# erlgo/openair4G

Measured on AMD Instinct MI355X. Metric: DL subframes/sec (20 MHz, 2x2, 64-QAM), higher is better.
Workload: dtype int16; 1 GPU; dlsim 20 MHz 2x2 TM3 (LARGE_CDD) 64-QAM MCS19x2CW, 2x14 IDFT-2048; config_id=C3, global_batch=8192, subframe_index=7, full_grid=False, parallelism=subframe-sharded x1

## Files before the change

include/oai4g.h:

```cpp
#ifndef OAI4G_H
#define OAI4G_H

#include <stddef.h>
#include <stdint.h>

#ifdef __cplusplus
extern "C" {
#endif

#define OAI4G_LTE_NULL 2
#define OAI4G_NSOFT 1827072
#define OAI4G_MAX_SEGMENTS 16
#define OAI4G_MAX_CHANNEL_BITS (14 * 1200 * 6)
#define OAI4G_D_BYTES (96 + 12 + 3 + 3 * 6144)
#define OAI4G_W_BYTES (3 * 6144 + 96)

enum { OAI4G_SISO = 0, OAI4G_ALAMOUTI = 1, OAI4G_LARGE_CDD = 2 };
enum { OAI4G_CYCLIC_PREFIX = 0, OAI4G_CYCLIC_SUFFIX = 1, OAI4G_ZEROS = 2, OAI4G_NONE = 3 };

typedef struct {
  uint16_t N_RB_DL;
  uint16_t Nid_cell;
  uint8_t Ncp;
  uint8_t nushift;
// ... 23 lines not shown
  uint32_t format;
  uint8_t dci_pdu[8];
} oai4g_dci_alloc_t;

typedef struct {
  uint32_t TBS;
  uint32_t B;
  uint8_t *b;
  uint8_t *c[OAI4G_MAX_SEGMENTS];
  uint32_t RTC[OAI4G_MAX_SEGMENTS];
  uint8_t round;
  uint8_t mcs;
  uint8_t rvidx;
  uint8_t mimo_mode;
  uint32_t rb_alloc[4];
  uint16_t nb_rb;
  uint8_t *e;
  uint8_t *d[OAI4G_MAX_SEGMENTS];
  uint8_t *w[OAI4G_MAX_SEGMENTS];
  uint32_t C, Cminus, Cplus, Kminus, Kplus, F;
  uint8_t Nl;
  uint8_t Nlayers;
  uint8_t first_layer;
} oai4g_dl_harq_t;

typedef struct {
  uint16_t rnti;
  uint8_t current_harq_pid;
  uint8_t Mdlharq;
  uint8_t Kmimo;
  int16_t sqrt_rho_a;
  int16_t sqrt_rho_b;
  oai4g_dl_harq_t *harq_processes[8];
} oai4g_dlsch_t;

int oai4g_init(void);
const char *oai4g_last_error(void);
int oai4g_device_name(char *buf, int len);

int oai4g_init_frame_parms(oai4g_frame_parms_t *fp, uint16_t N_RB_DL, uint16_t Nid_cell, uint8_t Ncp,
                           uint8_t nb_antennas_tx, uint8_t mode1_flag, uint8_t frame_type);
uint8_t oai4g_get_Qm(uint8_t mcs);
int oai4g_get_G(const oai4g_frame_parms_t *fp, uint16_t nb_rb, const uint32_t *rb_alloc, uint8_t mod_order,
                uint8_t Nl, uint8_t num_pdcch_symbols, int frame, uint8_t subframe);
uint8_t oai4g_get_Qm_ul(uint8_t mcs);
uint8_t oai4g_get_I_TBS(uint8_t mcs);
uint8_t oai4g_get_I_TBS_UL(uint8_t mcs);
uint32_t oai4g_tbs_bits(uint8_t I_TBS, uint16_t nb_rb);
uint32_t oai4g_get_TBS_DL(uint8_t mcs, uint16_t nb_rb);
uint32_t oai4g_get_TBS_UL(uint8_t mcs, uint16_t nb_rb);
oai4g_dlsch_t *oai4g_new_dlsch(uint8_t Kmimo, uint8_t Mdlharq, uint8_t N_RB_DL);
void oai4g_free_dlsch(oai4g_dlsch_t *dlsch);
uint32_t oai4g_lte_gold_generic(uint32_t *x1, uint32_t *x2, uint8_t reset);

uint32_t oai4g_crc24a(const uint8_t *in, int bitlen);
uint32_t oai4g_crc24b(const uint8_t *in, int bitlen);
int oai4g_lte_segmentation(const uint8_t *input_buffer, uint8_t **output_buffers, uint32_t B, uint32_t *C,
                           uint32_t *Cplus, uint32_t *Cminus, uint32_t *Kplus, uint32_t *Kminus, uint32_t *F);
void oai4g_threegpplte_turbo_encoder(const uint8_t *input, uint16_t input_length_bytes, uint8_t *output,
                                     uint8_t F, uint16_t interleaver_f1, uint16_t interleaver_f2);
uint32_t oai4g_sub_block_interleaving_turbo(uint32_t D, uint8_t *d, uint8_t *w);
uint32_t oai4g_lte_rate_matching_turbo(uint32_t RTC, uint32_t G, const uint8_t *w, uint8_t *e, uint8_t C,
                                       uint32_t Nsoft, uint8_t Mdlharq, uint8_t Kmimo, uint8_t rvidx,
                                       uint8_t Qm, uint8_t Nl, uint8_t r, uint8_t nb_rb, uint8_t m);
int oai4g_dlsch_encoding(uint8_t *a, const oai4g_frame_parms_t *frame_parms, uint8_t num_pdcch_symbols,
                         oai4g_dlsch_t *dlsch, int frame, uint8_t subframe);
void oai4g_dlsch_scrambling(const oai4g_frame_parms_t *frame_parms, int mbsfn_flag, oai4g_dlsch_t *dlsch, int G,
                            uint8_t q, uint8_t Ns);
int oai4g_dlsch_modulation(int32_t **txdataF, int16_t amp, uint32_t subframe_offset,
                           const oai4g_frame_parms_t *frame_parms, uint8_t num_pdcch_symbols,
                           oai4g_dlsch_t *dlsch0, oai4g_dlsch_t *dlsch1);
void oai4g_PHY_ofdm_mod(const int32_t *input, int32_t *output, uint8_t log2fftsize, uint8_t nb_symbols,
                        uint16_t nb_prefix_samples, int etype);
void oai4g_normal_prefix_mod(const int32_t *txdataF, int32_t *txdata, uint8_t nsymb,
                             const oai4g_frame_parms_t *frame_parms);
void oai4g_do_OFDM_mod(int32_t **txdataF, int32_t **txdata, uint32_t frame, uint16_t next_slot,
                       const oai4g_frame_parms_t *frame_parms);
void oai4g_generate_pilots(int32_t **txdataF, int16_t amp, const oai4g_frame_parms_t *frame_parms, uint16_t Ntti);
int oai4g_lte_dl_cell_spec(int32_t *output, int16_t amp, const oai4g_frame_parms_t *frame_parms, uint8_t Ns,
                           uint8_t l, uint8_t p);
int oai4g_idft(int log2n, const int16_t *x, int16_t *y, int scale);
void oai4g_idft2048(const int16_t *x, int16_t *y, int scale);
void oai4g_idft1024(const int16_t *x, int16_t *y, int scale);
void oai4g_idft512(const int16_t *x, int16_t *y, int scale);
void oai4g_idft256(const int16_t *x, int16_t *y, int scale);
void oai4g_idft128(const int16_t *x, int16_t *y, int scale);
void oai4g_idft64(const int16_t *x, int16_t *y, int scale);

void oai4g_generate_pcfich_reg_mapping(const oai4g_frame_parms_t *frame_parms, uint16_t pcfich_reg[4],
                                       uint8_t *pcfich_first_reg_idx);
int oai4g_generate_pcfich(uint8_t num_pdcch_symbols, int16_t amp, const oai4g_frame_parms_t *frame_parms,
                          int32_t **txdataF, uint8_t subframe);

uint8_t oai4g_get_mi(const oai4g_frame_parms_t *frame_parms, uint8_t subframe);
uint16_t oai4g_get_nquad(uint8_t num_pdcch_symbols, const oai4g_frame_parms_t *frame_parms, uint8_t mi);
uint16_t oai4g_get_nCCE(uint8_t num_pdcch_symbols, const oai4g_frame_parms_t *frame_parms, uint8_t mi);
uint8_t oai4g_get_num_pdcch_symbols(uint8_t num_dci, const oai4g_dci_alloc_t *dci_alloc,
                                    const oai4g_frame_parms_t *frame_parms, uint8_t subframe);
int oai4g_generate_phich_reg_mapping(const oai4g_frame_parms_t *frame_parms, uint16_t phich_reg[56][3]);
void oai4g_init_nCCE_table(void);
int oai4g_get_nCCE_offset(uint8_t L, int nCCE, int common_dci, uint16_t rnti, uint8_t subframe);
uint8_t oai4g_generate_dci_top(uint8_t num_ue_spec_dci, uint8_t num_common_dci, const oai4g_dci_alloc_t *dci_alloc,
                               uint32_t n_rnti, int16_t amp, const oai4g_frame_parms_t *frame_parms,
                               int32_t **txdataF, uint32_t subframe);

int oai4g_rx_pdsch_siso(const oai4g_frame_parms_t *frame_parms, const int32_t *rxdataF, const int32_t *dl_ch_estimates,
// ... 234 lines not shown
```

openair4g_amd/__init__.py:

```python
import ctypes
import os

import numpy as np

_HERE = os.path.dirname(os.path.abspath(__file__))
LIB_PATH = os.path.join(_HERE, "lib", "libopenair4g_amd.so")

LTE_NULL = 2
NSOFT = 1827072
MAX_SEGMENTS = 16
MAX_CHANNEL_BITS = 14 * 1200 * 6
D_BYTES = 96 + 12 + 3 + 3 * 6144
W_BYTES = 3 * 6144 + 96
SISO, ALAMOUTI, LARGE_CDD = 0, 1, 2
CYCLIC_PREFIX = 0


class OAI4GError(RuntimeError):
    pass


u8p = ctypes.POINTER(ctypes.c_uint8)


# ... 243 lines not shown
                                                 ctypes.c_uint8, ctypes.c_uint32, ctypes.c_uint8]),
    "oai4g_ul_config_destroy": (None, [ctypes.c_void_p]),
    "oai4g_ul_config_C": (ctypes.c_int, [ctypes.c_void_p]),
    "oai4g_ul_config_E": (ctypes.c_uint32, [ctypes.c_void_p, ctypes.c_int]),
    "oai4g_ul_config_G_offset": (ctypes.c_uint32, [ctypes.c_void_p, ctypes.c_int]),
    "oai4g_ul_decode_batch": (ctypes.c_int, [ctypes.c_void_p, ctypes.c_int, ctypes.c_void_p, ctypes.c_size_t,
                                             ctypes.c_void_p, ctypes.c_size_t, ctypes.c_void_p, ctypes.c_void_p]),
    "oai4g_ul_config_w_entries": (ctypes.c_size_t, [ctypes.c_void_p]),
    "oai4g_ul_decode_batch_harq": (ctypes.c_int, [ctypes.c_void_p, ctypes.c_int, ctypes.c_void_p, ctypes.c_size_t,
                                                  ctypes.c_void_p, ctypes.c_size_t, ctypes.c_uint8, ctypes.c_uint8,
                                                  ctypes.c_void_p, ctypes.c_size_t, ctypes.c_void_p, ctypes.c_void_p]),
    "oai4g_dft": (ctypes.c_int, [ctypes.c_int, ctypes.c_void_p, ctypes.c_void_p, ctypes.c_int]),
    "oai4g_dft2048": (None, [ctypes.c_void_p, ctypes.c_void_p, ctypes.c_int]),
    "oai4g_dft1024": (None, [ctypes.c_void_p, ctypes.c_void_p, ctypes.c_int]),
    "oai4g_dft512": (None, [ctypes.c_void_p, ctypes.c_void_p, ctypes.c_int]),
    "oai4g_dft256": (None, [ctypes.c_void_p, ctypes.c_void_p, ctypes.c_int]),
    "oai4g_dft128": (None, [ctypes.c_void_p, ctypes.c_void_p, ctypes.c_int]),
    "oai4g_dft64": (None, [ctypes.c_void_p, ctypes.c_void_p, ctypes.c_int]),
    "oai4g_slot_fep_offset": (ctypes.c_int64, [ctypes.POINTER(FrameParms), ctypes.c_uint8, ctypes.c_uint8,
                                               ctypes.c_int, ctypes.c_int]),
    "oai4g_slot_fep": (ctypes.c_int, [ctypes.POINTER(ctypes.c_void_p), ctypes.POINTER(ctypes.c_void_p),
                                      ctypes.POINTER(FrameParms), ctypes.c_uint8, ctypes.c_uint8, ctypes.c_uint8,
                                      ctypes.c_int, ctypes.c_int]),
    "oai4g_fep_batch": (ctypes.c_int, [ctypes.POINTER(FrameParms), ctypes.c_int, ctypes.c_int, ctypes.c_void_p,
                                       ctypes.c_void_p, ctypes.c_void_p]),
    "oai4g_tx_config_create": (ctypes.c_void_p, [ctypes.POINTER(TxParams)]),
    "oai4g_tx_config_destroy": (None, [ctypes.c_void_p]),
    "oai4g_tx_G": (ctypes.c_uint32, [ctypes.c_void_p, ctypes.c_int, ctypes.c_int]),
    "oai4g_tx_ebits_words": (ctypes.c_uint32, [ctypes.c_void_p]),
    "oai4g_tx_iq_samples": (ctypes.c_uint32, [ctypes.c_void_p]),
    "oai4g_tx_workspace_bytes": (ctypes.c_size_t, [ctypes.c_void_p, ctypes.c_int]),
    "oai4g_tx_batch": (ctypes.c_int, [ctypes.c_void_p, ctypes.c_int, ctypes.c_void_p, ctypes.c_void_p,
                                      ctypes.c_void_p, ctypes.c_void_p]),
    "oai4g_tx_batch_timed": (ctypes.c_int, [ctypes.c_void_p, ctypes.c_int, ctypes.c_void_p, ctypes.c_void_p,
                                            ctypes.c_void_p, ctypes.c_void_p, ctypes.POINTER(ctypes.c_float)]),
    "oai4g_tx_encode": (ctypes.c_int, [ctypes.c_void_p, ctypes.c_int, ctypes.c_void_p, ctypes.c_void_p,
                                       ctypes.c_void_p]),
    "oai4g_tx_modulate": (ctypes.c_int, [ctypes.c_void_p, ctypes.c_int, ctypes.c_void_p, ctypes.c_void_p,
                                         ctypes.c_void_p]),
    "oai4g_tx_mod_nosat": (ctypes.c_int, [ctypes.c_void_p]),
    "oai4g_diag_encode_phase_ms": (ctypes.c_int, [ctypes.c_void_p, ctypes.c_int, ctypes.c_void_p, ctypes.c_void_p,
                                                  ctypes.c_int, ctypes.c_int, ctypes.POINTER(ctypes.c_float)]),
    "oai4g_diag_encode_occupancy": (ctypes.c_int, [ctypes.c_void_p, ctypes.POINTER(ctypes.c_int),
                                                   ctypes.POINTER(ctypes.c_size_t)]),
    "oai4g_diag_stream": (ctypes.c_int, [ctypes.c_void_p, ctypes.c_void_p, ctypes.c_size_t, ctypes.c_int,
                                         ctypes.c_void_p]),
    "oai4g_dev_alloc": (ctypes.c_void_p, [ctypes.c_size_t]),
    "oai4g_dev_free": (None, [ctypes.c_void_p]),
    "oai4g_memcpy_h2d": (ctypes.c_int, [ctypes.c_void_p, ctypes.c_void_p, ctypes.c_size_t]),
    "oai4g_memcpy_d2h": (ctypes.c_int, [ctypes.c_void_p, ctypes.c_void_p, ctypes.c_size_t]),
    "oai4g_memset_d": (ctypes.c_int, [ctypes.c_void_p, ctypes.c_int, ctypes.c_size_t]),
    "oai4g_sync": (ctypes.c_int, []),
    "oai4g_fill_payload": (ctypes.c_int, [ctypes.c_void_p, ctypes.c_size_t, ctypes.c_uint64, ctypes.c_void_p]),
}


def load_library(path=None):
    global _lib
    if _lib is not None:
        return _lib
    path = path or os.environ.get("OAI4G_LIB") or LIB_PATH
    if not os.path.exists(path):
        raise OAI4GError(f"HIP library not built: {path} (run __graft_entry__.build())")
    lib = ctypes.CDLL(path)
    for name, (res, args) in _SIGS.items():
        fn = getattr(lib, name)
        fn.restype = res
        fn.argtypes = args
    _lib = lib
    return lib


def exported_symbols():
    return sorted(_SIGS)


def lib():
    return load_library()


def init():
    L = lib()
    if L.oai4g_init() != 0:
        raise OAI4GError(L.oai4g_last_error().decode())
    return L


def _check(ok):
    if not ok:
        raise OAI4GError(lib().oai4g_last_error().decode())


def _ptr(a):
    return ctypes.c_void_p(a.ctypes.data)


def device_name():
    L = init()
    buf = ctypes.create_string_buffer(256)
    _check(L.oai4g_device_name(buf, 256) == 0)
    return buf.value.decode()


def frame_parms(N_RB_DL, Nid_cell=0, Ncp=0, nb_antennas_tx=1, mode1_flag=1, frame_type=0):
    fp = FrameParms()
    _check(lib().oai4g_init_frame_parms(ctypes.byref(fp), N_RB_DL, Nid_cell, Ncp, nb_antennas_tx, mode1_flag,
# ... 1005 lines not shown
```

openair4g_amd/csrc/oai4g_encode.hip:

```cpp
#include "oai4g_internal.h"

struct rsc_tables_t {
  uint8_t next[8][16];
  uint8_t par[8][16];
  uint8_t apow[8][8];
  uint32_t hz;
  uint32_t zs[8];
  uint32_t fm[3];
};

static constexpr uint8_t rsc_step_c(uint8_t u, uint8_t s, uint8_t *out)
{
  *out = (uint8_t)((u ^ (s >> 2) ^ (s >> 1)) & 1);
  return (uint8_t)((((u << 2) ^ (s >> 1)) ^ ((s >> 1) << 2) ^ (s << 2)) & 7);
}

static constexpr rsc_tables_t make_rsc_tables()
{
  rsc_tables_t t{};
  for (int s = 0; s < 8; s++)
    for (int nib = 0; nib < 16; nib++) {
      uint8_t st = (uint8_t)s, p = 0;
      for (int b = 0; b < 4; b++) {
        uint8_t o = 0;
// ... 585 lines not shown
  if (DEBUG && dbg.b)
    for (uint32_t i = tid; i < Ab + 3; i += nth) dbg.b[i] = tbb[i];
  if (stop_phase <= 1) return;

  for (uint32_t i = tid; i < C * 3 * 4; i += nth) {
    const uint32_t slot = i >> 2, r = slot / 3;
    const uint32_t w = (r < n0 ? kw0 : kw1) + (i & 3u);
    if (w < sw) strm[slot * sw + w] = 0u;
  }
  auto unit_of = [&](uint32_t i, uint32_t &r, uint32_t &j, uint32_t &K, uint32_t &ki) {
    ki = i >= u0 ? 1u : 0u;
    const uint32_t ii = ki ? i - u0 : i, kw = ki ? kw1 : kw0;
    const uint32_t rr = __umul24(ii, ki ? km1 : km0) >> 20;
    j = ii - __umul24(rr, kw);
    r = ki ? n0 + rr : rr;
    K = ki ? kk1 : kk0;
  };
  for (uint32_t i = tid; i < nw; i += nth) {
    uint32_t r, j, K, ki;
    unit_of(i, r, j, K, ki);
    uint32_t fill, ncopy, s0;
    seg_of(r, fill, ncopy, s0);
    const uint32_t i0 = 4 * j;
    uint32_t le;
    if (i0 >= fill) {
      const uint32_t a = s0 + i0 - fill, wi = a >> 2;
      le = __builtin_amdgcn_alignbit(tbw[wi + 1], tbw[wi], (a & 3u) * 8u);
      const int sh = (int)(fill + ncopy) - (int)i0;
      if (C > 1 && sh < 4) {
        const uint32_t crcle = __builtin_bswap32(crcs[1 + r] << 8);
        const uint32_t cw32 = (uint32_t)(((uint64_t)crcle << (8 * (sh + 4))) >> 32);
        le = (sh > 0 ? le & (0xffffffffu >> (32 - 8 * sh)) : 0u) | cw32;
      }
    } else {
      const uint32_t crcb = C > 1 ? crcs[1 + r] : 0;
      le = 0;
      for (uint32_t q = 0; q < 4; q++) {
        const uint32_t ib = i0 + q;
        uint32_t byte = 0;
        if (ib < fill) byte = 0;
        else if (ib < fill + ncopy) byte = tbb[s0 + ib - fill];
        else if (C > 1 && ib < fill + ncopy + 3) byte = (crcb >> (8 * (2 - (ib - fill - ncopy)))) & 0xffu;
        le |= byte << (8 * q);
      }
    }
    uint32_t wv = bytes_to_seq(le);
    if (32 * (j + 1) > K) wv &= (1u << (K - 32 * j)) - 1u;
    strm[r * 3 * sw + j] = wv;
  }
  __syncthreads();
  if (stop_phase <= 2) return;

  uint32_t *ilv = lds_base;
  for (uint32_t r = 0; r < C; r++) {
    const uint32_t K = r < n0 ? kk0 : kk1, Kw = (K + 31) >> 5, Q = K >> 2, io = r < n0 ? r * kw0 : u0 + (r - n0) * kw1;
    const uint32_t *sys = strm + r * 3 * sw;
    for (uint32_t w = tid; w < Kw; w += nth) ilv[io + w] = 0u;
    const uint32_t ng = (Q + 31) >> 5, nbw = (Q + 7) >> 3;
    for (uint32_t g = tid; g < ng; g += nth) {
      uint32_t P[4];
#pragma unroll
      for (uint32_t q = 0; q < 4; q++) {
        const uint32_t src = 32 * g + q * Q, wi = src >> 5;
        const uint32_t lo = sys[wi], hi = wi + 1 < Kw ? sys[wi + 1] : 0u;
        uint32_t v = __builtin_amdgcn_alignbit(hi, lo, src);
        if (src + 32 > K) v |= sys[0] << (K - src);
        P[q] = v;
      }
#pragma unroll
      for (uint32_t jb = 0; jb < 4; jb++) {
        const uint32_t t01 = __builtin_amdgcn_perm(P[1], P[0], 0x0c0c0000u | jb | ((4 + jb) << 8));
        const uint32_t t23 = __builtin_amdgcn_perm(P[3], P[2], 0x00000c0cu | (jb << 16) | ((4 + jb) << 24));
        if (4 * g + jb < nbw) strm[(r * 3 + 1) * sw + 4 * g + jb] = t01 | t23;
      }
    }
  }
  __syncthreads();
  {
    const bool s3a = __builtin_amdgcn_readfirstlane(cw.qpp_s3[0]) != 0, s3b = __builtin_amdgcn_readfirstlane(cw.qpp_s3[1]) != 0;
    for (uint32_t i = tid; i < nw; i += nth) {
      uint32_t r, j, K, ki;
      unit_of(i, r, j, K, ki);
      const uint32_t Q = K >> 2;
      const uint4 e4 = *(const uint4 *)&cw.qpp_tab[ki][4 * j];
      const uint32_t ew[4] = {e4.x, e4.y, e4.z, e4.w};
      const uint32_t *b8 = strm + (r * 3 + 1) * sw;
      uint32_t acc = 0;
#pragma unroll
      for (int b = 0; b < 8; b++) {
        const uint32_t e = (b & 1) ? ew[b >> 1] >> 16 : ew[b >> 1];
        const uint32_t D = *(const uint32_t *)((const uint8_t *)b8 + __builtin_amdgcn_ubfe(e, 5, 10));
        acc |= __builtin_amdgcn_alignbit(D, D, e) & (0x01010101u << b);
      }
      uint32_t a0 = acc & 0xffu, a1 = (acc >> 8) & 0xffu, a2 = (acc >> 16) & 0xffu, a3 = acc >> 24;
      const uint32_t n = Q - 8 * j;
      if (n < 8) {
        const uint32_t m = (1u << n) - 1u;
        a0 &= m; a1 &= m; a2 &= m; a3 &= m;
      }
      const bool s3 = ki ? s3b : s3a;
      const uint32_t q1 = s3 ? a3 : a1, q3 = s3 ? a1 : a3;
      uint32_t *o = ilv + (i - j);
      if ((Q & 7u) == 0) {
        uint8_t *ob = (uint8_t *)o + j;
        const uint32_t qb = Q >> 3;
        ob[0] = (uint8_t)a0; ob[qb] = (uint8_t)q1; ob[2 * qb] = (uint8_t)a2; ob[3 * qb] = (uint8_t)q3;
      } else {
        or_bits(o, 8 * j, a0);
        or_bits(o, Q + 8 * j, q1);
        or_bits(o, 2 * Q + 8 * j, a2);
        or_bits(o, 3 * Q + 8 * j, q3);
      }
    }
  }
  __syncthreads();
  if (stop_phase == 23) return;

  for (uint32_t seg = wave; seg < 2 * C; seg += nwaves) {
    const uint32_t r = seg >> 1, e = seg & 1u;
    uint32_t *blk = strm + r * 3 * sw;
    const uint32_t io = r < n0 ? r * kw0 : u0 + (r - n0) * kw1;
    turbo_segment(e ? ilv + io : blk, blk + (1 + e) * sw, r < n0 ? kk0 : kk1, &tails[2 * r + e], tabs);
  }
  __syncthreads();
  if (stop_phase <= 3) return;

  if (DEBUG) {
    for (uint32_t r = 0; r < C; r++) {
      uint32_t K = cw.K[r], R = cw.R[r], Kpi = cw.Kpi[r], ND = cw.ND[r];
      const uint32_t *blk = strm + r * 3 * sw;
      if (dbg.c)
        for (uint32_t i = tid; i < K / 8; i += nth) {
          uint32_t wv = blk[(i >> 2)];
// ... 121 lines not shown
          const uint32_t ro = rob;
          if constexpr (decltype(ONCE)::value) {
            const int l = min((int)m, (int)E - (int)o);
            if (l > 0) or_bits2(ebuf, ro + o, y & (0xffffffffu >> (32 - l)));
            if (wtc - t0 < 2u) {
              asm volatile("" ::: "memory");
              if (dst & OAI4G_RM_DST_WRAP) {
                const uint32_t ma = Nnn - o;
                const uint32_t l2 = min(m - ma, E);
                or_bits2(ebuf, ro, (y >> ma) & (0xffffffffu >> (32 - l2)));
              }
            }
          } else if (m) {
            y &= 0xffffffffu >> (32 - m);
            const uint32_t ma = min(m, Nnn - o);
            for (uint32_t part = 0; part < 2; part++) {
              const uint32_t len = part ? m - ma : ma, os = part ? 0u : o;
              const uint32_t v = part ? (ma < 32 ? y >> ma : 0u) : (ma < 32 ? y & ((1u << ma) - 1u) : y);
              for (uint32_t x = os; len && x < E; x += Nnn) {
                const uint32_t l = min(len, E - x);
                or_bits(ebuf, ro + x, v & (0xffffffffu >> (32 - l)));
              }
            }
          }
          if (r2 != r) enter(r2, k2);
          ki = k2;
          r = r2;
          t0 = t2;
        }
      };
      if (once) pair_loop(std::true_type{});
      else pair_loop(std::false_type{});
      __syncthreads();
      if (DEBUG) {
        for (uint32_t k = tid; k < G; k += nth) dbg.e[k] = (uint8_t)((ebuf[k >> 5] >> (k & 31)) & 1u);
        return;
      }
      const uint32_t nst = stop_phase <= 4 ? 0u : ((h + 1 < nhalf && (eb1 & 31u)) ? nwh - 1 : nwh);
      for (uint32_t i = tid; i < nst; i += nth) {
        const uint32_t wi = w0 + i;
        uint32_t v = ebuf[i] ^ gold[wi];
        const uint32_t nb = min(32u, G - 32 * wi);
        if (nb < 32) v &= (1u << nb) - 1u;
        eout[wi] = v;
      }
      if (h + 1 < nhalf) {
        carry = (eb1 & 31u) ? ebuf[nwh - 1] : 0u;
        __syncthreads();
      }
    }
  }
}

__global__ void __launch_bounds__(256) k_encode(const cfg_dev_t *__restrict__ c, const uint8_t *__restrict__ payload,
                                                uint32_t *__restrict__ ebits, int stop_phase, uint32_t sf0)
{
  extern __shared__ uint32_t lds_dyn[];
  uint32_t sf = blockIdx.x / c->n_cw, cwi = blockIdx.x % c->n_cw;
  enc_debug_t none = {nullptr, nullptr, nullptr, nullptr, nullptr};
  encode_codeword<false>(c, sf, cwi, payload, ebits, none, lds_dyn, stop_phase, sf0);
}

__global__ void __launch_bounds__(256) k_encode_debug(const cfg_dev_t *__restrict__ c, uint32_t sf, uint32_t cwi,
                                                      const uint8_t *__restrict__ payload, enc_debug_t dbg)
{
  extern __shared__ uint32_t lds_dyn[];
  encode_codeword<true>(c, sf, cwi, payload, nullptr, dbg, lds_dyn);
}

static size_t enc_lds_bytes(const cfg_dev_t *h)
{
  size_t words = (size_t)h->lds_a_words + h->lds_b_words + 2 * OAI4G_MAX_CB + OAI4G_MAX_CB + 2 + 4;
  size_t bytes = words * 4 + sizeof(enc_tabs_t);
#ifdef OAI4G_ENC_LDS_PAD
  bytes += OAI4G_ENC_LDS_PAD;
#endif
  return (bytes + 15) & ~(size_t)15;
}

static hipError_t launch_encode_impl(const cfg_dev_t *d_cfg, const cfg_dev_t *h_cfg, int sf0, int n_sf,
                                     const uint8_t *d_payload, uint32_t *d_ebits, int stop_phase, hipStream_t s);

hipError_t oai4g_launch_encode(const cfg_dev_t *d_cfg, const cfg_dev_t *h_cfg, int sf0, int n_sf,
                               const uint8_t *d_payload, uint32_t *d_ebits, hipStream_t s)
{
  return launch_encode_impl(d_cfg, h_cfg, sf0, n_sf, d_payload, d_ebits, 99, s);
}

hipError_t oai4g_launch_encode_phase(const cfg_dev_t *d_cfg, const cfg_dev_t *h_cfg, int n_sf,
                                     const uint8_t *d_payload, uint32_t *d_ebits, int stop_phase, hipStream_t s)
{
  return launch_encode_impl(d_cfg, h_cfg, 0, n_sf, d_payload, d_ebits, stop_phase, s);
}

static hipError_t launch_encode_impl(const cfg_dev_t *d_cfg, const cfg_dev_t *h_cfg, int sf0, int n_sf,
                                     const uint8_t *d_payload, uint32_t *d_ebits, int stop_phase, hipStream_t s)
{
  if (n_sf <= 0) return hipSuccess;
  d_payload += (size_t)sf0 * h_cfg->n_cw * h_cfg->payload_stride;
  d_ebits += (size_t)sf0 * h_cfg->n_cw * h_cfg->ebits_words;
  size_t lds = enc_lds_bytes(h_cfg);
  static bool attr_set = false;
  if (!attr_set) {
    (void)hipFuncSetAttribute((const void *)k_encode, hipFuncAttributeMaxDynamicSharedMemorySize, 160 * 1024);
    (void)hipFuncSetAttribute((const void *)k_encode_debug, hipFuncAttributeMaxDynamicSharedMemorySize, 160 * 1024);
    attr_set = true;
  }
// ... 224 lines not shown
```

openair4g_amd/csrc/oai4g_host.cpp:

```cpp
#include <hip/hip_runtime.h>
#include <math.h>
#include <pthread.h>
#include <stdarg.h>
#include <stdio.h>
#include <stdlib.h>
#include <string.h>

#include <algorithm>
#include <cmath>
#include <cstdlib>
#include <vector>
#include <map>
#include <mutex>
#include <vector>

#include "../../include/oai4g.h"
#include "../../include/oai4g_qpp.h"
#include "../../include/oai4g_tbs.h"
#include "oai4g_internal.h"

static thread_local char g_err[512] = "";

static void set_err(const char *fmt, ...)
{
// ... 626 lines not shown
  int re_alloc[10];
  hipStream_t s_mod = nullptr;
  hipEvent_t ev_enc[OAI4G_PIPE_MAX_CHUNKS] = {};
  hipEvent_t ev_done = nullptr;
  int pipe_chunk = 0;
};

static void rm_plan(cw_dev_t &c, int ki)
{
  const uint32_t R = c.Rk[ki], ND = c.NDk[ki], Ncb = c.Ncbk[ki], Nnn = c.Nnnk[ki], k0c = c.k0ck[ki];
  const uint32_t tz = c.t0k[ki], nt = c.ntk[ki], sw = c.stream_words;
  memset(c.rm_dst[ki], 0, sizeof(c.rm_dst[ki]));
  c.rm_wrapt[ki] = ~0u;
  for (uint32_t t = 0; t <= OAI4G_RM_TILES; t++)
    for (uint32_t L = 0; L < 32; L++) c.rm_src[ki][t][L] = 1u << 5;
  for (uint32_t t = 0; t < nt; t++) {
    const bool il = t >= tz;
    const uint32_t rb = il ? t - tz : t;
    for (uint32_t L = 0; L < 32; L++) {
      const uint32_t row = il ? 16 * rb + (L >> 1) : 32 * rb + L, s = il ? 1 + (L & 1) : 0;
      if (row < R) {
        const int pos = (int)(32 * row) - (int)ND + (s == 2 ? 1 : 0);
        const uint32_t wrel = (uint32_t)((int)(s * sw) + (pos >> 5) + 1);
        c.rm_src[ki][t][L] = ((uint32_t)pos & 31u) | (wrel << 5) | (s == 2 && row == R - 1 ? OAI4G_RM_SRC_LAST : 0u);
      }
      uint32_t wc = 0;
      for (int b = 0; b < 5; b++) wc |= ((L >> b) & 1u) << (4 - b);
      uint32_t b0 = 0, b1 = 0;
      for (uint32_t w2 = 0; w2 < wc; w2++) {
        uint32_t p2 = 0;
        for (int b = 0; b < 5; b++) p2 |= ((w2 >> b) & 1u) << (4 - b);
        b0 += p2 < ND ? 1u : 0u;
        b1 += p2 + 1 < ND ? 1u : 0u;
      }
      const uint32_t z0 = L < ND ? 1u : 0u, z1 = z0 + (L + 1 < ND ? 1u : 0u);
      const uint32_t zc = il ? z1 : z0;
      const uint32_t cs = il ? 32 * R - ND + 2 * wc * R - b0 - b1 : wc * R - b0;
      const uint32_t pc = il ? 32 * R + 2 * wc * R : wc * R;
      const int left = il ? 2 * ((int)R - 16 * (int)rb) : (int)R - 32 * (int)rb;
      int n = left < 32 ? left : 32;
      if (il && L == 31 && ND > 0 && left <= 32 && n) n--;
      const uint32_t z = rb ? 0u : zc, ci0 = rb ? cs + 32 * rb - zc : cs, p0 = pc + 32 * rb;
      const int m = p0 + (uint32_t)n > Ncb ? (int)Ncb - (int)(p0 + z) : n - (int)z;
      if (m <= 0) continue;
      uint32_t o = ci0 + Nnn - k0c;
      o = o >= Nnn ? o - Nnn : o;
      c.rm_dst[ki][t][L] = o | (z << 16) | ((uint32_t)m << 21) | (o + (uint32_t)m > Nnn ? OAI4G_RM_DST_WRAP : 0u);
      if (o + (uint32_t)m > Nnn) c.rm_wrapt[ki] = c.rm_wrapt[ki] == ~0u || c.rm_wrapt[ki] == t ? t : ~1u;
    }
  }
  if (getenv("OAI4G_ENC_GENERAL_RM")) c.rm_wrapt[ki] = ~1u;
}

static int derive_cfg(oai4g_tx_config *cfg, const oai4g_tx_params_t *p, const uint8_t Nl[2], bool need_remap,
                      int only_sf)
{
  memset(&cfg->h, 0, sizeof(cfg->h));
  cfg->p = *p;
  oai4g_frame_parms_t &fp = cfg->fp;
  if (oai4g_init_frame_parms(&fp, p->N_RB_DL, p->Nid_cell, p->Ncp, p->nb_antennas_tx, p->mode1_flag,
                             p->frame_type) != 0)
    return -1;
  cfg_dev_t &h = cfg->h;
  if (p->n_cw < 1 || p->n_cw > 2) { set_err("n_cw must be 1 or 2"); return -1; }
  if (p->mimo_mode != OAI4G_SISO && p->mimo_mode != OAI4G_LARGE_CDD && p->mimo_mode != OAI4G_ALAMOUTI) {
    set_err("mimo_mode %u not supported (SISO, ALAMOUTI and LARGE_CDD)", p->mimo_mode);
    return -1;
  }
  if (p->mimo_mode == OAI4G_ALAMOUTI && (p->nb_antennas_tx != 2 || p->n_cw != 1)) {
    set_err("ALAMOUTI requires 2 TX antennas and one codeword (dlsch_modulation.c:362)");
    return -1;
  }
  if (p->mimo_mode == OAI4G_LARGE_CDD && ((p->nb_antennas_tx != 2 && p->nb_antennas_tx != 4) || p->n_cw != 2)) {
    set_err("LARGE_CDD requires 2 (dlsch_modulation.c:551) or 4 (C4 extension) TX antennas and 2 codewords");
    return -1;
  }
  if (p->nb_antennas_tx == 4 && p->mimo_mode != OAI4G_LARGE_CDD) {
    set_err("4 TX antennas: LARGE_CDD only (C4 extension)");
    return -1;
  }
  if (p->payload_stride % 4) { set_err("payload_stride must be a multiple of 4"); return -1; }
  h.N_RB_DL = fp.N_RB_DL;
  h.N = fp.ofdm_symbol_size;
  h.log2N = fp.log2_symbol_size;
  h.cp0 = fp.nb_prefix_samples0;
  h.cp = fp.nb_prefix_samples;
  h.spt = fp.samples_per_tti;
  h.nsymb = fp.symbols_per_tti;
  h.n_ant = fp.nb_antennas_tx;
  h.first_carrier = fp.first_carrier_offset;
  h.n_cw = p->n_cw;
  h.mimo_mode = p->mimo_mode;
  h.num_pdcch = p->num_pdcch_symbols;
  h.rnti = p->rnti;
  h.Nid_cell = p->Nid_cell;
  h.first_sf = p->first_subframe % 10;
  h.sf_step = p->subframe_step;
  h.payload_stride = p->payload_stride;
  for (uint32_t v = 0; v < 256; v++) {
    uint32_t ra = v << 16, rb = v << 16;
    for (int i = 0; i < 8; i++) {
      ra = (ra & 0x800000u) ? ((ra << 1) ^ 0x864cfbu) & 0xffffffu : (ra << 1) & 0xffffffu;
      rb = (rb & 0x800000u) ? ((rb << 1) ^ 0x800063u) & 0xffffffu : (rb << 1) & 0xffffffu;
    }
    h.crctab[0][v] = ra;
    h.crctab[1][v] = rb;
// ... 2 lines not shown
  bool rm_fail = false;
  for (int cw = 0; cw < p->n_cw; cw++) {
    cw_dev_t &c = h.cw[cw];
    c.TBS = p->TBS[cw];
    if (c.TBS == 0 || (c.TBS & 7)) { set_err("TBS[%d]=%u must be a positive multiple of 8", cw, c.TBS); return -1; }
    c.A_bytes = c.TBS >> 3;
    if (p->payload_stride < ((c.A_bytes + 3) & ~3u)) {
      set_err("payload_stride %u < TBS/8 rounded to 4 (%u)", p->payload_stride, (c.A_bytes + 3) & ~3u);
      return -1;
    }
    c.Qm = oai4g_get_Qm(p->mcs[cw]);
    c.q = p->q[cw];
    uint32_t C, Cp, Cm, Kp, Km, F, L;
    if (seg_params(c.TBS + 24, &C, &Cp, &Cm, &Kp, &Km, &F, &L) < 0) { set_err("segmentation failed"); return -1; }
    c.C = C; c.Cminus = Cm; c.Kplus = Kp; c.Kminus = Km; c.F = F; c.L = L;
    uint32_t src = 0, maxK = 0;
    for (uint32_t r = 0; r < C; r++) {
      uint32_t K = r < Cm ? Km : Kp;
      int qi = oai4g_qpp_index(K);
      if (qi < 0) { set_err("illegal code block size %u", K); return -1; }
      c.K[r] = K;
      c.f1[r] = oai4g_qpp_table[qi].f1;
      c.f2[r] = oai4g_qpp_table[qi].f2;
      c.fill[r] = r == 0 ? F / 8 : 0;
      c.ncopy[r] = (K - L) / 8 - c.fill[r];
      c.src[r] = src;
      src += c.ncopy[r];
      maxK = K > maxK ? K : maxK;
      uint32_t D = K + 4, R = (D + 31) >> 5, Kpi = R << 5;
      c.R[r] = R; c.Kpi[r] = Kpi; c.ND[r] = Kpi - D;
      uint32_t Kw = 3 * Kpi;
      uint32_t Nir = OAI4G_NSOFT / p->Kmimo / (p->Mdlharq < 8 ? p->Mdlharq : 8);
      uint32_t Ncb = (Nir / C < Kw) ? Nir / C : Kw;
      if (Ncb < Kw && !p->rm_limited_buffer) {
        printf("Exiting, RM condition (Nir %u, Nsoft %u, Kw %u\n", Nir, OAI4G_NSOFT, Kw);
        set_err("RM condition: Ncb %u < Kw %u (the reference emits E=0, lte_rate_matching.c:518-521)", Ncb, Kw);
        rm_fail = true;
        Ncb = Kw;
      }
      c.Ncb[r] = Ncb;
      c.kidx[r] = (C > 1 && r < Cm) ? 0 : 1;
    }
    if (src != (c.TBS + 24) / 8) { set_err("segmentation byte accounting mismatch"); return -1; }
    for (int ki = 0; ki < 2; ki++) {
      uint32_t K = ki == 0 ? Km : Kp;
      if (K == 0 || (ki == 0 && !(C > 1 && Cm > 0))) continue;
      int qi = oai4g_qpp_index(K);
      uint64_t f1 = oai4g_qpp_table[qi].f1, f2 = oai4g_qpp_table[qi].f2;
      for (uint32_t j = 0; j < (K + 31) / 32; j++) {
        uint64_t k = 8 * j;
        uint32_t pi = (uint32_t)((f1 * k + f2 * k * k) % K), pi1 = (uint32_t)((f1 * (k + 1) + f2 * (k + 1) * (k + 1)) % K);
        c.qpp0[ki][j] = pi | (((pi1 + K - pi) % K) << 16);
      }
      c.qpp_d2[ki] = (uint32_t)((2 * f2) % K);
      memset(c.qpp_tab[ki], 0, sizeof(c.qpp_tab[ki]));
      for (uint64_t k = 0; k < K / 4; k++) {
        const uint32_t x = (uint32_t)((f1 * k + f2 * k * k) % K), Q = K / 4, xp = x % Q, u = x / Q;
        const uint32_t rot = (8 * u + (xp & 7) + 32 - (uint32_t)(k & 7)) & 31u;
        c.qpp_tab[ki][k >> 1] |= (((xp >> 3) << 7) | rot) << (16 * (k & 1));
      }
      c.qpp_s3[ki] = (uint32_t)((f1 * (K / 4)) % K) == K / 4 ? 0u : 1u;
    }
    {
      uint32_t o = 0;
      for (uint32_t r = 0; r < C; r++) {
        c.ilv_off[r] = o;
        o += (c.K[r] + 31) / 32;
      }
      c.ilv_off[C] = o;
      c.n0 = (C > 1) ? Cm : 0;
      c.kk[0] = c.n0 ? Km : Kp;
      c.kk[1] = Kp;
      for (int ki = 0; ki < 2; ki++) {
        c.kw[ki] = (c.kk[ki] + 31) / 32;
        c.kmag[ki] = ((1u << 20) + c.kw[ki] - 1) / c.kw[ki];
      }
      c.u0 = c.n0 * c.kw[0];
    }
    c.crc_per_tb = (((c.A_bytes + 255) / 256) + 3) & ~3u;
    crc_mul_tables(c.crc_per_tb, 8, 0x864cfbu, c.crcmul_tb);
    crc_mul_tables2(c.crc_per_tb, 0x864cfbu, c.crc2_tb);
    uint32_t ncb_max = 0;
    for (uint32_t r = 0; r < C; r++) {
      uint32_t n = c.ncopy[r];
      if (c.src[r] + n > c.A_bytes) n = c.A_bytes > c.src[r] ? c.A_bytes - c.src[r] : 0;
      ncb_max = n > ncb_max ? n : ncb_max;
    }
    c.crc_lpb = C <= 4 ? 64u : (C <= 8 ? 32u : 16u);
    c.crc_per_cb = (((ncb_max + c.crc_lpb - 1) / c.crc_lpb) + 3) & ~3u;
    crc_mul_tables2(c.crc_per_cb ? c.crc_per_cb : 1, 0x864cfbu, c.crc2_cb[0]);
    crc_mul_tables2(c.crc_per_cb ? c.crc_per_cb : 1, 0x800063u, c.crc2_cb[1]);
    for (uint32_t r = 0; r < C; r++) {
      uint32_t end = c.src[r] + c.ncopy[r];
      if (end > c.A_bytes) end = c.A_bytes;
      const uint32_t m = crc_xpow8_h(c.A_bytes - (end > c.src[r] ? end : c.src[r]), 0x864cfbu);
      for (int k = 0; k < 6; k++)
        for (uint32_t v = 0; v < 16; v++) c.crcmul_blk[r][16 * k + v] = crc_mulmod_h((v << (4 * k)) & 0xffffffu, m, 0x864cfbu);
    }
    for (int ki = 0; ki < 2; ki++) {
      uint32_t K = ki == 0 ? (Km ? Km : Kp) : Kp;
      int n = null_positions(K, c.nullpos[ki], OAI4G_MAX_NULLS);
      if (n < 0) { set_err("too many NULL positions"); return -1; }
      c.nnull[ki] = (uint32_t)n;
    }
    for (uint32_t r = 0; r < C; r++) {
      uint32_t R = c.R[r], Ncb = c.Ncb[r], nn = c.nnull[c.kidx[r]];
      const uint16_t *np = c.nullpos[c.kidx[r]];
      uint32_t ncol8 = R << 3;
      uint32_t k0 = R * (2 + p->rvidx[cw] * ((Ncb % ncol8 ? 1 : 0) + Ncb / ncol8) * 2);
      uint32_t before = 0, inbuf = 0;
      for (uint32_t i = 0; i < nn; i++) {
        if (np[i] < k0) before++;
        if (np[i] < Ncb) inbuf++;
      }
// ... 3311 lines not shown
```

openair4g_amd/csrc/oai4g_internal.h:

```cpp
#pragma once
#include <hip/hip_runtime.h>
#include <stdint.h>

#include "../../include/oai4g.h"

#define OAI4G_MAX_CB 16
#define OAI4G_MAX_NULLS 104
#define OAI4G_MAX_CHUNKS 192
#define OAI4G_MAX_TASKS (OAI4G_MAX_CB * 20)
#define OAI4G_RM_TILES 20
#define OAI4G_RM_SRC_LAST (1u << 20)
#define OAI4G_RM_DST_WRAP (1u << 27)
#define OAI4G_PIPE_MAX_CHUNKS 16
#define OAI4G_CRS_CODE 0xE000u
#define OAI4G_CTL_CODE 0xC000u
static constexpr uint32_t oai4g_mod_entry_shift(uint32_t mimo_mode, uint32_t n_ant, uint32_t log2N)
{
  return log2N != 11 ? 1u : mimo_mode == OAI4G_LARGE_CDD && n_ant == 2 ? 3u : mimo_mode == OAI4G_SISO ? 2u : 1u;
}
static constexpr uint32_t oai4g_mod_addr_mask(uint32_t shift) { return 0x7FFFu & ~((1u << shift) - 1u); }
static constexpr uint32_t oai4g_mod_sentinel(uint32_t N) { return (3u * N) / 4u; }
static constexpr bool oai4g_mod_nre_fits(uint32_t nre, uint32_t N) { return nre + 3u <= oai4g_mod_sentinel(N); }
#define OAI4G_ENC_CRC_TABLE_WORDS (256 + 256)
#define OAI4G_GOLD_LANES 256
#define OAI4G_GOLD_STRIDE 17
#define OAI4G_MAX_GOLD_WORDS (OAI4G_GOLD_LANES * OAI4G_GOLD_STRIDE)
#define OAI4G_TW_TOTAL (16 + 64 + 128 + 256 + 512 + 1024 + 2048)

static inline __host__ __device__ uint32_t oai4g_tw_offset(int log2s)
{
  switch (log2s) {
  case 4: return 0;
  case 6: return 16;
  case 7: return 80;
  case 8: return 208;
  case 9: return 464;
  case 10: return 976;
  case 11: return 2000;
  default: return 0;
  }
}

struct cw_dev_t {
  uint32_t TBS;
  uint32_t A_bytes;
  uint32_t C, Cminus, Kplus, Kminus, F, L;
  uint32_t Qm;
  uint32_t q;
  uint32_t K[OAI4G_MAX_CB];
  uint32_t f1[OAI4G_MAX_CB], f2[OAI4G_MAX_CB];
  uint32_t src[OAI4G_MAX_CB];
  uint32_t fill[OAI4G_MAX_CB];
  uint32_t ncopy[OAI4G_MAX_CB];
  uint32_t crc_off[OAI4G_MAX_CB];
  uint32_t R[OAI4G_MAX_CB], Kpi[OAI4G_MAX_CB], ND[OAI4G_MAX_CB], Ncb[OAI4G_MAX_CB];
  uint32_t Nnn[OAI4G_MAX_CB];
  uint32_t k0c[OAI4G_MAX_CB];
  uint32_t kidx[OAI4G_MAX_CB];
  uint32_t wpk_off[OAI4G_MAX_CB + 1];
  uint32_t ntask;
  uint16_t tasks[OAI4G_MAX_TASKS];
  uint32_t ilv_off[OAI4G_MAX_CB + 1];
  uint32_t qpp0[2][OAI4G_MAX_CHUNKS];
  alignas(16) uint32_t qpp_tab[2][OAI4G_MAX_CHUNKS * 4];
  uint32_t qpp_d2[2];
  uint32_t qpp_s3[2];
  uint32_t n0, u0, kk[2], kw[2], kmag[2];
  uint32_t Rk[2], NDk[2], Ncbk[2], Nnnk[2], k0ck[2];
  uint32_t ntk[2], t0k[2], ntmag[2];
  uint32_t rm_wrapt[2];
  uint32_t nullcol[2][2];
  uint32_t esplit[10], ew[10][2], emag[10][2];
  uint32_t nnull[2];
  uint16_t nullpos[2][OAI4G_MAX_NULLS];
  uint32_t G[10];
  uint32_t E[10][OAI4G_MAX_CB];
  uint32_t roff[10][OAI4G_MAX_CB + 1];
  int16_t qam_a[8], qam_b[8];
  int16_t qpsk_a, qpsk_b;
  int16_t alm_qpsk[2][2];
  uint32_t stream_words;
  uint32_t crc_per_tb;
  uint32_t crc_per_cb;
  uint32_t crc_lpb;
  uint32_t crcmul_tb[8][6][16];
  uint32_t crcmul_blk[OAI4G_MAX_CB][96];
  uint32_t crc2_tb[2][8][96];
  uint32_t crc2_cb[2][2][8][96];
  uint32_t rm_src[2][OAI4G_RM_TILES + 1][32];
  uint32_t rm_dst[2][OAI4G_RM_TILES + 1][32];
};

struct cfg_dev_t {
  uint32_t N_RB_DL, N, log2N, cp0, cp, spt, nsymb, n_ant, first_carrier;
  uint32_t n_cw, mimo_mode, num_pdcch, rnti, Nid_cell, first_sf, sf_step;
  uint32_t payload_stride;
  uint32_t ebits_words;
  uint32_t lds_tb_words;
  uint32_t lds_stream_words;
  uint32_t lds_gold_words;
  uint32_t lds_w_words;
  uint32_t lds_a_words;
  uint32_t lds_b_words;
  uint32_t mod_nosat;
  uint32_t pad;
  uint32_t crctab[2][256];
  cw_dev_t cw[2];
  uint32_t symbase[10][14];
  uint32_t symnre[10][14];
  uint32_t n_cu;
  const uint16_t *remap;
  const uint16_t *remap_tm;
  uint32_t with_crs;
  uint32_t pilmask;
  uint32_t ctlmask[10];
  uint32_t ctl_on;
  const uint32_t *gold_tab;
  const uint32_t *gold_x1;
// ... 226 lines not shown
```

Before: 8.549 million subframes/s.

## Add 32-fold QPP interleaver fast path using bit-transpose tiles

Adds a host check for turbo block sizes that are multiples of 1024 whose QPP interleaver splits into 32 cosets with a constant odd stride. For those code blocks the encode kernel builds the interleaved systematic stream by transposing 32x32 bit tiles and using a per-row rotation table, in place of the generic per-unit gather path. It also caps the kernel's scalar register count with an attribute. The cost targeted is the interleaver gather in the encode kernel; the trade-off is extra LDS scratch traffic and two more code paths, and only block sizes that pass the fold test use the new path.

```diff
diff --git a/include/oai4g.h b/include/oai4g.h
--- a/include/oai4g.h
+++ b/include/oai4g.h
@@ -99,6 +99,7 @@
 oai4g_dlsch_t *oai4g_new_dlsch(uint8_t Kmimo, uint8_t Mdlharq, uint8_t N_RB_DL);
 void oai4g_free_dlsch(oai4g_dlsch_t *dlsch);
 uint32_t oai4g_lte_gold_generic(uint32_t *x1, uint32_t *x2, uint8_t reset);
+int oai4g_qpp_fold32(uint32_t K, uint32_t *s, uint16_t *tab);
 
 uint32_t oai4g_crc24a(const uint8_t *in, int bitlen);
 uint32_t oai4g_crc24b(const uint8_t *in, int bitlen);
diff --git a/openair4g_amd/__init__.py b/openair4g_amd/__init__.py
--- a/openair4g_amd/__init__.py
+++ b/openair4g_amd/__init__.py
@@ -319,6 +319,7 @@
     "oai4g_memset_d": (ctypes.c_int, [ctypes.c_void_p, ctypes.c_int, ctypes.c_size_t]),
     "oai4g_sync": (ctypes.c_int, []),
     "oai4g_fill_payload": (ctypes.c_int, [ctypes.c_void_p, ctypes.c_size_t, ctypes.c_uint64, ctypes.c_void_p]),
+    "oai4g_qpp_fold32": (ctypes.c_int, [ctypes.c_uint32, ctypes.POINTER(ctypes.c_uint32), ctypes.c_void_p]),
 }
 
 
diff --git a/openair4g_amd/csrc/oai4g_encode.hip b/openair4g_amd/csrc/oai4g_encode.hip
--- a/openair4g_amd/csrc/oai4g_encode.hip
+++ b/openair4g_amd/csrc/oai4g_encode.hip
@@ -661,7 +661,38 @@
   if (stop_phase <= 2) return;
 
   uint32_t *ilv = lds_base;
+  const uint32_t fw0 = __builtin_amdgcn_readfirstlane(cw.qpp_f32[0]), fw1 = __builtin_amdgcn_readfirstlane(cw.qpp_f32[1]);
+  const bool f32a = n0 != 0 && fw0 != 0, f32b = fw1 != 0;
+  const uint32_t ft0 = f32a ? n0 * (kw0 >> 5) : 0u, ftn = ft0 + (f32b ? (C - n0) * (kw1 >> 5) : 0u);
+  const uint32_t fm0 = fw0 >> 5, fm1 = fw1 >> 5;
+  uint32_t *etab0 = strm + 2 * sw, *etab1 = strm + (n0 * 3 + 2) * sw;
+  uint32_t te0 = 0, te1 = 0;
+  if (f32a && tid < kw0) te0 = ((const uint16_t *)cw.qpp_tab[0])[tid];
+  if (f32b && tid < kw1) te1 = ((const uint16_t *)cw.qpp_tab[1])[tid];
+  auto tile_of = [&](uint32_t i, uint32_t &r, uint32_t &t, uint32_t &nt, uint32_t &ki) {
+    ki = i >= ft0 ? 1u : 0u;
+    const uint32_t ii = ki ? i - ft0 : i;
+    nt = (ki ? kw1 : kw0) >> 5;
+    const uint32_t rr = __umul24(ii, ki ? fm1 : fm0) >> 20;
+    t = ii - __umul24(rr, nt);
+    r = ki ? n0 + rr : rr;
+  };
+  if (ftn) {
+    const tp_lane_t tpl = tp_lane(tid & 31);
+    const uint32_t l32 = tid & 31u;
+    const uint32_t sa = fw0 & 31u, sb = fw1 & 31u;
+    for (uint32_t base = 0; base < ftn; base += nth >> 5) {
+      uint32_t r, t, nt, ki;
+      tile_of(min(base + (tid >> 5), ftn - 1), r, t, nt, ki);
+      uint32_t *sys = strm + r * 3 * sw;
+      const uint32_t v = sys[t + nt * (((ki ? sb : sa) * l32) & 31u)];
+      sys[sw + 32 * t + l32] = transpose32_t<0>(v, tpl);
+    }
+    if (f32a && tid < kw0) etab0[tid] = te0;
+    if (f32b && tid < kw1) etab1[tid] = te1;
+  }
   for (uint32_t r = 0; r < C; r++) {
+    if (r < n0 ? f32a : f32b) continue;
     const uint32_t K = r < n0 ? kk0 : kk1, Kw = (K + 31) >> 5, Q = K >> 2, io = r < n0 ? r * kw0 : u0 + (r - n0) * kw1;
     const uint32_t *sys = strm + r * 3 * sw;
     for (uint32_t w = tid; w < Kw; w += nth) ilv[io + w] = 0u;
@@ -685,9 +716,23 @@
     }
   }
   __syncthreads();
+  if (ftn) {
+    const tp_lane_t tpl = tp_lane(tid & 31);
+    const uint32_t l32 = tid & 31u;
+    for (uint32_t base = 0; base < ftn; base += nth >> 5) {
+      uint32_t r, t, nt, ki;
+      tile_of(min(base + (tid >> 5), ftn - 1), r, t, nt, ki);
+      const uint32_t e = (ki ? etab1 : etab0)[32 * t + l32];
+      const uint32_t *T = strm + (r * 3 + 1) * sw;
+      const uint32_t D = *(const uint32_t *)((const uint8_t *)T + __builtin_amdgcn_ubfe(e, 5, 10));
+      const uint32_t io = r < n0 ? r * kw0 : u0 + (r - n0) * kw1;
+      ilv[io + t + nt * l32] = transpose32_t<0>(__builtin_amdgcn_alignbit(D, D, e), tpl);
+    }
+  }
   {
     const bool s3a = __builtin_amdgcn_readfirstlane(cw.qpp_s3[0]) != 0, s3b = __builtin_amdgcn_readfirstlane(cw.qpp_s3[1]) != 0;
-    for (uint32_t i = tid; i < nw; i += nth) {
+    const uint32_t ulo = f32a ? u0 : 0u, uhi = f32b ? u0 : nw;
+    for (uint32_t i = ulo + tid; i < uhi; i += nth) {
       uint32_t r, j, K, ki;
       unit_of(i, r, j, K, ki);
       const uint32_t Q = K >> 2;
@@ -915,7 +960,7 @@
   }
 }
 
-__global__ void __launch_bounds__(256) k_encode(const cfg_dev_t *__restrict__ c, const uint8_t *__restrict__ payload,
+__global__ void __launch_bounds__(256) __attribute__((amdgpu_num_sgpr(80))) k_encode(const cfg_dev_t *__restrict__ c, const uint8_t *__restrict__ payload,
                                                 uint32_t *__restrict__ ebits, int stop_phase, uint32_t sf0)
 {
   extern __shared__ uint32_t lds_dyn[];
diff --git a/openair4g_amd/csrc/oai4g_host.cpp b/openair4g_amd/csrc/oai4g_host.cpp
--- a/openair4g_amd/csrc/oai4g_host.cpp
+++ b/openair4g_amd/csrc/oai4g_host.cpp
@@ -702,6 +702,30 @@
   if (getenv("OAI4G_ENC_GENERAL_RM")) c.rm_wrapt[ki] = ~1u;
 }
 
+extern "C" int oai4g_qpp_fold32(uint32_t K, uint32_t *s_out, uint16_t *tab)
+{
+  const int qi = oai4g_qpp_index(K);
+  if (qi < 0 || oai4g_qpp_table[qi].K != K) return -1;
+  if (K & 1023u) return 0;
+  const uint64_t f1 = oai4g_qpp_table[qi].f1, f2 = oai4g_qpp_table[qi].f2;
+  const uint32_t Q = K >> 5;
+  auto pi = [&](uint64_t k) { return (uint32_t)((f1 * k + f2 * k * k) % K); };
+  const uint32_t d = (pi(Q) + K - pi(0)) % K;
+  if (d % Q) return 0;
+  const uint32_t s = d / Q;
+  if (!(s & 1u)) return 0;
+  for (uint32_t k = 0; k < K; k++)
+    if ((pi(k + Q) + K - pi(k)) % K != d) return 0;
+  uint32_t si = 1;
+  while (((si * s) & 31u) != 1u) si += 2;
+  *s_out = s;
+  for (uint32_t k = 0; k < Q; k++) {
+    const uint32_t x = pi(k);
+    tab[k] = (uint16_t)(((x % Q) << 7) | ((si * (x / Q)) & 31u));
+  }
+  return 1;
+}
+
 static int derive_cfg(oai4g_tx_config *cfg, const oai4g_tx_params_t *p, const uint8_t Nl[2], bool need_remap,
                       int only_sf)
 {
@@ -810,7 +834,6 @@
         uint32_t pi = (uint32_t)((f1 * k + f2 * k * k) % K), pi1 = (uint32_t)((f1 * (k + 1) + f2 * (k + 1) * (k + 1)) % K);
         c.qpp0[ki][j] = pi | (((pi1 + K - pi) % K) << 16);
       }
-      c.qpp_d2[ki] = (uint32_t)((2 * f2) % K);
       memset(c.qpp_tab[ki], 0, sizeof(c.qpp_tab[ki]));
       for (uint64_t k = 0; k < K / 4; k++) {
         const uint32_t x = (uint32_t)((f1 * k + f2 * k * k) % K), Q = K / 4, xp = x % Q, u = x / Q;
@@ -818,6 +841,14 @@
         c.qpp_tab[ki][k >> 1] |= (((xp >> 3) << 7) | rot) << (16 * (k & 1));
       }
       c.qpp_s3[ki] = (uint32_t)((f1 * (K / 4)) % K) == K / 4 ? 0u : 1u;
+      static_assert(sizeof(c.qpp_tab[0]) >= OAI4G_MAX_CHUNKS * sizeof(uint16_t), "32-fold entries fit qpp_tab");
+      uint32_t s32 = 0;
+      uint16_t t32[OAI4G_MAX_CHUNKS];
+      if (oai4g_qpp_fold32(K, &s32, t32) == 1) {
+        memset(c.qpp_tab[ki], 0, sizeof(c.qpp_tab[ki]));
+        memcpy(c.qpp_tab[ki], t32, (K / 32) * sizeof(uint16_t));
+        c.qpp_f32[ki] = s32 | ((((1u << 20) + K / 1024 - 1) / (K / 1024)) << 5);
+      }
     }
     {
       uint32_t o = 0;
diff --git a/openair4g_amd/csrc/oai4g_internal.h b/openair4g_amd/csrc/oai4g_internal.h
--- a/openair4g_amd/csrc/oai4g_internal.h
+++ b/openair4g_amd/csrc/oai4g_internal.h
@@ -63,7 +63,7 @@
   uint32_t ilv_off[OAI4G_MAX_CB + 1];
   uint32_t qpp0[2][OAI4G_MAX_CHUNKS];
   alignas(16) uint32_t qpp_tab[2][OAI4G_MAX_CHUNKS * 4];
-  uint32_t qpp_d2[2];
+  uint32_t qpp_f32[2];
   uint32_t qpp_s3[2];
   uint32_t n0, u0, kk[2], kw[2], kmag[2];
   uint32_t Rk[2], NDk[2], Ncbk[2], Nnnk[2], k0ck[2];
```

New measurement: 8.826 million subframes/s (median of 6 runs). +3.2%, better.
